# jynik/OOKiedokie

Measured on AMD Instinct MI355X. Metric: IQ Msamples/s demodulated (SC16Q11->bits), higher is better.
Workload: dtype f32

## Files before the change

### include/ookiedokie_amd.h

```cpp
#ifndef OOKIEDOKIE_AMD_H
#define OOKIEDOKIE_AMD_H

#include <limits.h>
#include <stddef.h>
#include <stdint.h>

#ifdef __cplusplus
extern "C" {
#endif

#define OOKD_API_VERSION 1

#define OOKD_FILE_EOF INT_MIN

enum {
    OOKD_OK = 0,
    OOKD_ERR_ARG = -1,
    OOKD_ERR_IO = -2,
    OOKD_ERR_PARSE = -3,
    OOKD_ERR_HIP = -4,
    OOKD_ERR_CAPACITY = -5,
    OOKD_ERR_NOMEM = -6
};

// ... 170 lines not shown
                           uint64_t capture_stride_samples);

int ookd_rx_submit_device(ookd_rx *rx, const void *d_iq,
                          uint32_t num_captures,
                          uint64_t samples_per_capture,
                          uint64_t capture_stride_samples);
int ookd_rx_wait(ookd_rx *rx);

int ookd_rx_process_host(ookd_rx *rx, const int16_t *iq,
                         uint64_t num_samples);

int ookd_rx_shard_begin(ookd_rx *rx, const void *d_iq, uint64_t num_samples,
                        const int16_t *halo, uint64_t halo_samples,
                        int last_shard, const ookd_fsm_state *state_in,
                        ookd_fsm_state *state_out);
int ookd_rx_shard_refine(ookd_rx *rx, const ookd_fsm_state *state_in,
                         ookd_fsm_state *state_out);
uint64_t ookd_rx_halo_samples(const ookd_rx *rx);

int ookd_scan_domain_info(const ookd_device *device,
                          uint32_t samples_per_buffer,
                          uint32_t total_decimation, uint32_t out[8]);

uint64_t ookd_rx_num_messages(const ookd_rx *rx);
const ookd_message *ookd_rx_messages(const ookd_rx *rx);
int ookd_rx_get_stats(const ookd_rx *rx, ookd_rx_stats *out);
int ookd_rx_get_front_info(const ookd_rx *rx, ookd_front_info *out);

uint64_t ookd_rx_bit_words(const ookd_rx *rx);
int ookd_rx_get_bits(const ookd_rx *rx, uint32_t capture, uint64_t *words,
                     uint64_t capacity_words);
int ookd_rx_get_edges(const ookd_rx *rx, uint32_t capture, uint64_t *edges,
                      uint64_t capacity, uint64_t *num_edges);
int ookd_rx_get_fir(const ookd_rx *rx, uint32_t capture, ookd_complexf *out,
                    uint64_t capacity);
int ookd_rx_get_errors(const ookd_rx *rx, uint64_t *samples, uint64_t capacity,
                       uint64_t *num);

size_t ookd_rx_dig_text(const ookd_rx *rx, uint32_t capture, char *out, size_t capacity);
int ookd_rx_record_dig(const ookd_rx *rx, uint32_t capture, const char *path);
int ookd_rx_get_fir_sc16q11(const ookd_rx *rx, uint32_t capture, int16_t *out,
                            uint64_t capacity_samples);
int ookd_rx_record_fir(const ookd_rx *rx, uint32_t capture, const char *path);

#define OOKD_LEVEL_BINS 256
typedef struct ookd_level_hist {
// ... 157 lines not shown
```

### ookiedokie_amd/__init__.py

```python
from __future__ import annotations

import ctypes as C
import os
from dataclasses import dataclass
from typing import List, Optional, Sequence, Tuple

import numpy as np

_HERE = os.path.dirname(os.path.abspath(__file__))
LIB_PATH = os.path.join(_HERE, "lib", "libookiedokie_amd.so")
HEADER_PATH = os.path.join(_HERE, "..", "include", "ookiedokie_amd.h")

MAX_PAYLOAD_BYTES = 32
FILE_EOF = -(2 ** 31)
RX_EXACT_FIR = 1
RX_KEEP_FIR = 2
RX_FSM_ROUNDS = 4
RX_NO_QUIET_SKIP = 8
RX_COUNT_QUIET = 16
RX_SCAN_SIMS = 32
RX_NO_PIPELINE = 128
RX_FIR_VALU = 256
RX_SCAN_TABLES = 512
RX_SAMPLES_CS8 = 1024
# ... 151 lines not shown
    "ookd_filter_load": (C.c_void_p, [C.c_char_p]),
    "ookd_filter_create": (C.c_void_p, [C.c_uint32, C.c_void_p, C.c_void_p, C.c_void_p]),
    "ookd_filter_free": (None, [C.c_void_p]),
    "ookd_filter_total_decimation": (C.c_uint32, [C.c_void_p]),
    "ookd_filter_num_stages": (C.c_uint32, [C.c_void_p]),
    "ookd_filter_stage": (C.c_int, [C.c_void_p, C.c_uint32, C.POINTER(C.c_uint32),
                                    C.POINTER(C.c_uint32), C.POINTER(C.POINTER(C.c_float))]),
    "ookd_filter_tuned_taps": (C.c_int, [C.c_void_p, C.c_double, C.c_uint32, C.c_void_p, C.c_void_p]),
    "ookd_device_load": (C.c_void_p, [C.c_char_p, C.c_uint32]),
    "ookd_device_create": (C.c_void_p, [C.POINTER(FsmTables)]),
    "ookd_device_free": (None, [C.c_void_p]),
    "ookd_device_num_bits": (C.c_uint32, [C.c_void_p]),
    "ookd_device_name": (C.c_char_p, [C.c_void_p]),
    "ookd_device_state_name": (C.c_char_p, [C.c_void_p, C.c_uint32]),
    "ookd_device_tables": (C.c_int, [C.c_void_p, C.POINTER(FsmTables)]),
    "ookd_rx_create": (C.c_void_p, [C.POINTER(RxConfig), C.c_void_p, C.c_void_p]),
    "ookd_rx_create_tuned": (C.c_void_p, [C.POINTER(RxConfig), C.c_void_p, C.c_void_p, C.POINTER(Tune)]),
    "ookd_rx_tune": (C.c_double, [C.c_void_p]),
    "ookd_rx_destroy": (None, [C.c_void_p]),
    "ookd_rx_sample_bytes": (C.c_uint32, [C.c_void_p]),
    "ookd_rx_process_device": (C.c_int, [C.c_void_p, C.c_void_p, C.c_uint32, C.c_uint64, C.c_uint64]),
    "ookd_rx_submit_device": (C.c_int, [C.c_void_p, C.c_void_p, C.c_uint32, C.c_uint64, C.c_uint64]),
    "ookd_scan_domain_info": (C.c_int, [C.c_void_p, C.c_uint32, C.c_uint32, C.POINTER(C.c_uint32)]),
    "ookd_rx_wait": (C.c_int, [C.c_void_p]),
    "ookd_rx_process_host": (C.c_int, [C.c_void_p, C.c_void_p, C.c_uint64]),
    "ookd_rx_shard_begin": (C.c_int, [C.c_void_p, C.c_void_p, C.c_uint64, C.c_void_p, C.c_uint64,
                                      C.c_int, C.POINTER(FsmState), C.POINTER(FsmState)]),
    "ookd_rx_shard_refine": (C.c_int, [C.c_void_p, C.POINTER(FsmState), C.POINTER(FsmState)]),
    "ookd_rx_halo_samples": (C.c_uint64, [C.c_void_p]),
    "ookd_rx_num_messages": (C.c_uint64, [C.c_void_p]),
    "ookd_rx_messages": (C.POINTER(Message), [C.c_void_p]),
    "ookd_rx_get_stats": (C.c_int, [C.c_void_p, C.POINTER(RxStats)]),
    "ookd_rx_get_front_info": (C.c_int, [C.c_void_p, C.POINTER(FrontInfo)]),
    "ookd_rx_bit_words": (C.c_uint64, [C.c_void_p]),
    "ookd_rx_get_bits": (C.c_int, [C.c_void_p, C.c_uint32, C.c_void_p, C.c_uint64]),
    "ookd_rx_get_edges": (C.c_int, [C.c_void_p, C.c_uint32, C.c_void_p, C.c_uint64,
                                    C.POINTER(C.c_uint64)]),
    "ookd_rx_get_fir": (C.c_int, [C.c_void_p, C.c_uint32, C.c_void_p, C.c_uint64]),
    "ookd_rx_get_errors": (C.c_int, [C.c_void_p, C.c_void_p, C.c_uint64, C.POINTER(C.c_uint64)]),
    "ookd_fir_create": (C.c_void_p, [C.c_int32, C.c_void_p, C.c_size_t, C.c_uint32]),
    "ookd_fir_reset": (None, [C.c_void_p]),
    "ookd_fir_destroy": (None, [C.c_void_p]),
    "ookd_fir_filter_and_decimate": (C.c_size_t, [C.c_void_p, C.c_void_p, C.c_size_t, C.c_void_p]),
    "ookd_synth_create": (C.c_void_p, [C.c_void_p, C.POINTER(SynthConfig), C.c_uint64]),
    "ookd_synth_free": (None, [C.c_void_p]),
    "ookd_synth_num_messages": (C.c_uint64, [C.c_void_p]),
# ... 843 lines not shown
```

### ookiedokie_amd/csrc/fir_mfma.hip

```cpp
#include "kernels.hpp"
#include "common.hpp"

#include <hip/hip_ext.h>

#include <algorithm>
#include <cmath>
#include <cstring>
#include <type_traits>

#pragma clang fp contract(off)

namespace ookd {

typedef _Float16 h8 __attribute__((ext_vector_type(8)));
typedef _Float16 h4 __attribute__((ext_vector_type(4)));
typedef float f16x __attribute__((ext_vector_type(16)));
typedef float v2fm __attribute__((ext_vector_type(2)));
typedef short v2s __attribute__((ext_vector_type(2)));
typedef uint32_t v4u __attribute__((ext_vector_type(4)));

__host__ __device__ constexpr uint32_t mslot(uint32_t j) { return j + 8u * (j >> 5); }

template <int KS, int FMT = (int)kFmtSc16>
struct MfmaGeom {
// ... 294 lines not shown
        are = __builtin_amdgcn_mfma_f32_32x32x16_f16(a1, xr, are, 0, 0, 0);
        aim = __builtin_amdgcn_mfma_f32_32x32x16_f16(a1, xi, aim, 0, 0, 0);
        __builtin_amdgcn_sched_barrier(0);
        xr = xr_n;
        xi = xi_n;
        a0 = a0_n;
        a1 = a1_n;
    }
    __builtin_amdgcn_fence(__ATOMIC_RELEASE, "wavefront");
    __builtin_amdgcn_wave_barrier();
}

template <int KS>
__device__ __noinline__ void mfma_fetch_image(const void *image, unsigned char *smem, uint32_t tid) {
    v4u *dst = reinterpret_cast<v4u *>(smem) + tid;
    const gptr128 src = reinterpret_cast<gptr128>((gbytes)image) + tid;
    for (int i = 0; i < 2 * KS; i += 4) {
        const v4u f0 = src[64 * i], f1 = src[64 * i + 64], f2 = src[64 * i + 128], f3 = src[64 * i + 192];
        dst[64 * i] = f0;
        dst[64 * i + 64] = f1;
        dst[64 * i + 128] = f2;
        dst[64 * i + 192] = f3;
    }
}

template <int KS, int FMT>
__global__ __launch_bounds__(64 * mfma_waves<KS>()) __attribute__((amdgpu_waves_per_eu(4)))
void fir1_mfma_kernel(const FrontParams p) {
    constexpr int kMfmaWaves = mfma_waves<KS>();
    extern __shared__ __attribute__((aligned(16))) unsigned char smem_raw[];
    using Gm = MfmaGeom<KS, FMT>;
    typedef typename RawSrcT<FMT>::elem raw_t;
    typedef typename RawSrcT<FMT>::ptr raw_ptr;
    constexpr uint32_t kImgBytes = (uint32_t)KS * 2u * 1024u;
    uint32_t tid = threadIdx.x & 63u;
    const uint32_t wave = threadIdx.x >> 6;
    const uint32_t cap = blockIdx.y;
    MfmaTileCtxT<FMT> c;
    c.rs.src = (raw_ptr)(reinterpret_cast<const raw_t *>(p.iq) + (uint64_t)cap * p.cap_stride);
    c.rs.halo = (raw_ptr)reinterpret_cast<const raw_t *>(p.halo);
    c.rs.halo_len = p.halo_len;
    c.rs.n_valid = p.n_valid;
    c.ctl = reinterpret_cast<uint32_t *>(smem_raw + kImgBytes);
    c.tickets = p.mfma_g * (uint32_t)kMfmaWaves;
    c.tile_base = p.tile_base;
    c.tile_end = p.tile_end;
// ... 61 lines not shown
                mfma_fetch_image<KS>(p.mfma_a, smem_raw, tid);
                __builtin_amdgcn_fence(__ATOMIC_RELEASE, "wavefront");
                __builtin_amdgcn_wave_barrier();
                if (tid == 0) __hip_atomic_store(&c.ctl[1], 1u, __ATOMIC_RELAXED, __HIP_MEMORY_SCOPE_WORKGROUP);
                __builtin_amdgcn_fence(__ATOMIC_ACQUIRE, "wavefront");
            }
            f16x are, aim;
            if (FMT != (int)kFmtSc16 || !wide) {
                mfma_convert<KS, FMT>(q, 0xffffffffu, tid, pl_re, pl_im);
                more = mfma_take_ticket(c, tid, tile_n);
                pre = more && mfma_interior<KS, FMT>(c, tile_n);
                if (pre) mfma_issue_loads<KS, FMT>(c, tile_n, tid, q);
                mfma_ksteps<KS, true>(a_img, pl_re, pl_im, tid, are, aim);
            } else if constexpr (FMT == (int)kFmtSc16) {
                mfma_convert<KS, FMT>(q, 0xffe0ffe0u, tid, pl_re, pl_im);
                mfma_ksteps<KS, true>(a_img, pl_re, pl_im, tid, are, aim);
                mfma_convert<KS, FMT>(q, 0x001f001fu, tid, pl_re, pl_im);
                more = mfma_take_ticket(c, tid, tile_n);
                pre = more && mfma_interior<KS, FMT>(c, tile_n);
                if (pre) mfma_issue_loads<KS, FMT>(c, tile_n, tid, q);
                mfma_ksteps<KS, false>(a_img, pl_re, pl_im, tid, are, aim);
            }

            const float plo = wide ? p.p_lo_w : p.p_lo_n;
            const float phi = wide ? p.p_hi_w : p.p_hi_n;
            const uint32_t ocol = 32u * n + 4u * hh;
            uint32_t m16 = 0;
            uint64_t any_unsure = 0;
#pragma unroll
            for (int r2 = 7; r2 >= 0; --r2) {
                const v2fm zr = (v2fm){are[2 * r2], are[2 * r2 + 1]}, zi = (v2fm){aim[2 * r2], aim[2 * r2 + 1]};
                const v2fm rr = zr * zr, ii = zi * zi;
                const v2fm pw = rr + ii;
                {
                    const uint64_t ge_hi = __ballot(pw.y >= phi);
                    asm("v_addc_co_u32_e64 %0, vcc, %0, %0, %1" : "+v"(m16) : "s"(ge_hi) : "vcc");
                    any_unsure |= __ballot(pw.y >= plo) & ~ge_hi;
                }
                {
                    const uint64_t ge_hi = __ballot(pw.x >= phi);
                    asm("v_addc_co_u32_e64 %0, vcc, %0, %0, %1" : "+v"(m16) : "s"(ge_hi) : "vcc");
                    any_unsure |= __ballot(pw.x >= plo) & ~ge_hi;
                }
            }
            if (any_unsure != 0) {
                uint32_t todo = 0, redo = 0;
#pragma unroll
                for (int r = 0; r < 16; ++r) {
                    const float rr = are[r] * are[r], ii = aim[r] * aim[r];
                    const float pw = rr + ii;
                    if (pw >= plo && !(pw >= phi)) todo |= 1u << r;
                }
                while (todo) {
                    const uint32_t r = (uint32_t)__ffs((int)todo) - 1u;
                    todo &= todo - 1u;
                    const uint64_t o = t0 + ocol + (r & 3u) + 8u * (r >> 2);
                    if (o >= p.n_out) continue;
                    const float2 y = mfma_exact_output(c.rs, (gptrf)p.taps, p.stage[0].ntaps, (int64_t)o);
                    const float rr = y.x * y.x, ii = y.y * y.y;
                    const float pe = rr + ii;
                    m16 = (m16 & ~(1u << r)) | ((pe >= p.p_star ? 1u : 0u) << r);
                    redo++;
                }
                if (redo && p.recompute_count) atomicAdd(p.recompute_count, (unsigned long long)redo);
            }
            if (fout) {
                const float cs = p.mfma_c;
#pragma unroll
                for (int r = 0; r < 16; ++r) {
                    const uint64_t o = t0 + ocol + (r & 3) + 8 * (r >> 2);
                    if (o < p.n_out) fout[o] = (v2fm){are[r] * cs, aim[r] * cs};
                }
            }

            uint32_t m32 = (m16 & 0xfu) | ((m16 & 0xf0u) << 4) | ((m16 & 0xf00u) << 8) | ((m16 & 0xf000u) << 12);
            m32 <<= 4u * hh;
            uint32_t w32 = m32 | (uint32_t)__shfl_xor((int)m32, 32);
            {
                const uint64_t c0 = t0 + 32u * n;
                if (c0 + 32u > p.n_out) {
                    const uint32_t keep = c0 >= p.n_out ? 0u : (uint32_t)(p.n_out - c0);
                    w32 &= (1u << keep) - 1u;
                }
            }
            {
                const uint32_t prev_top = (uint32_t)__shfl_up((int)(w32 >> 31), 1);
                uint32_t ch = w32 ^ (w32 << 1);
                if (n != 0) ch ^= prev_top & 1u;
                else ch &= ~1u;
                uint32_t cnt = hh == 0 ? (uint32_t)__popc(ch) : 0u;
#pragma unroll
                for (int d = 16; d >= 1; d >>= 1) cnt += (uint32_t)__shfl_xor((int)cnt, d);
                const uint32_t first = (uint32_t)__builtin_amdgcn_readfirstlane((int)(w32 & 1u));
                const uint32_t last = (uint32_t)__builtin_amdgcn_readlane((int)(w32 >> 31), 31);
                const uint64_t chl = __ballot(hh == 0 && ch != 0);
                const uint32_t widx = chl ? (uint32_t)__builtin_ctzll(chl) >> 1 : 0u;
                if (tid == 0) *uniform_ptr(tile_info + tile) = cnt | (widx << kTileWordShift) | (first << 30) | (last << 31) | p.stamp_bits;
            }
            const uint32_t up = (uint32_t)__shfl_xor((int)w32, 1);
            if (hh == 0 && (n & 1u) == 0) {
                const gbytes_w wb = uniform_ptr((gbytes_w)(words + (t0 >> 6)));
                *reinterpret_cast<gptr64>(wb + 4u * n) = (uint64_t)w32 | ((uint64_t)up << 32);
            }
        }

        if (!more) break;
        if (!pre) mfma_boundary_loads<KS, FMT>(c, tile_n, tid, win, q);
        tile = tile_n;
    }
}

constexpr uint32_t kF2Out = 256;
constexpr uint32_t kF2Tp = 96;
constexpr uint32_t kF2W = 4 * kF2Out + kF2Tp;
template <int FMT>
// ... 236 lines not shown
            if (__hip_atomic_load(&c.ctl[1], __ATOMIC_RELAXED, __HIP_MEMORY_SCOPE_WORKGROUP) == 0) {
                f2_fetch_image(p.mfma_a, smem_raw, tid);
                __builtin_amdgcn_fence(__ATOMIC_RELEASE, "wavefront");
                __builtin_amdgcn_wave_barrier();
                if (tid == 0) __hip_atomic_store(&c.ctl[1], 1u, __ATOMIC_RELAXED, __HIP_MEMORY_SCOPE_WORKGROUP);
                __builtin_amdgcn_fence(__ATOMIC_ACQUIRE, "wavefront");
            }
            f4x are, aim;
            if (FMT != (int)kFmtSc16 || !wide) {
                f2_convert<FMT>(q, 0xffffffffu, tid, pl_re, pl_im);
                more = mfma_take_ticket(c, tid, tile_n);
                pre = more && f2_interior(c, tile_n);
                if (pre) f2_issue_loads(c, tile_n, tid, q);
                f2_ksteps<true>(a_img, pl_re, pl_im, tid, are, aim);
            } else if constexpr (FMT == (int)kFmtSc16) {
                f2_convert<FMT>(q, 0xffe0ffe0u, tid, pl_re, pl_im);
                f2_ksteps<true>(a_img, pl_re, pl_im, tid, are, aim);
                f2_convert<FMT>(q, 0x001f001fu, tid, pl_re, pl_im);
                more = mfma_take_ticket(c, tid, tile_n);
                pre = more && f2_interior(c, tile_n);
                if (pre) f2_issue_loads(c, tile_n, tid, q);
                f2_ksteps<false>(a_img, pl_re, pl_im, tid, are, aim);
            }
            const float plo = wide ? p.p_lo_w : p.p_lo_n;
            const float phi = wide ? p.p_hi_w : p.p_hi_n;
            const uint32_t o_lane = 16u * n + 4u * g;
            uint32_t nib = 0, unsure = 0;
#pragma unroll
            for (int r = 0; r < 4; ++r) {
                const float rr = are[r] * are[r], ii = aim[r] * aim[r];
                const float pw = rr + ii;
                const bool hi = pw >= phi;
                nib |= (hi ? 1u : 0u) << r;
                unsure |= ((!hi && pw >= plo) ? 1u : 0u) << r;
            }
            if (__ballot(unsure != 0) != 0) {
                uint32_t todo = unsure, redo = 0;
                while (todo) {
                    const uint32_t r = (uint32_t)__ffs((int)todo) - 1u;
                    todo &= todo - 1u;
                    const uint64_t o = M0 + o_lane + r;
                    if (o >= p.n_out) continue;
                    const float2 y = fir2_mfma_exact_output(c.rs, ft, (int64_t)o);
                    const float rr = y.x * y.x, ii = y.y * y.y;
                    const float pe = rr + ii;
                    nib = (nib & ~(1u << r)) | ((pe >= p.p_star ? 1u : 0u) << r);
                    redo++;
                }
                if (redo && p.recompute_count) atomicAdd(p.recompute_count, (unsigned long long)redo);
            }
            if (fout) {
                const float cs = p.mfma_c;
#pragma unroll
                for (int r = 0; r < 4; ++r) {
                    const uint64_t o = M0 + o_lane + r;
                    if (o < p.n_out) fout[o] = (v2fm){are[r] * cs, aim[r] * cs};
                }
            }
            if (M0 + o_lane + 4u > p.n_out) {
                const uint32_t keep = M0 + o_lane >= p.n_out ? 0u : (uint32_t)(p.n_out - (M0 + o_lane));
                nib &= (1u << keep) - 1u;
            }
            uint64_t w64 = (uint64_t)nib << (16u * (n & 3u) + 4u * g);
#pragma unroll
            for (int d = 1; d <= 32; d <<= 1) {
                if (d == 4 || d == 8) continue;
                const uint32_t lo = (uint32_t)__shfl_xor((int)(uint32_t)w64, d), hi = (uint32_t)__shfl_xor((int)(uint32_t)(w64 >> 32), d);
                w64 |= (uint64_t)lo | ((uint64_t)hi << 32);
            }
            {
                const uint32_t wq = n >> 2;
                const uint32_t top_prev = (uint32_t)__shfl((int)(uint32_t)(w64 >> 63), (int)((wq ? wq - 1u : 0u) << 2));
                uint64_t ch = w64 ^ ((w64 << 1) | (wq ? (uint64_t)(top_prev & 1u) : 0ull));
                if (wq == 0) ch &= ~1ull;
                uint32_t cnt = ((n & 3u) == 0 && g == 0) ? (uint32_t)__popcll(ch) : 0u;
#pragma unroll
                for (int d = 32; d >= 1; d >>= 1) cnt += (uint32_t)__shfl_xor((int)cnt, d);
                const uint32_t first = (uint32_t)__builtin_amdgcn_readfirstlane((int)(uint32_t)(w64 & 1ull));
                const uint32_t last = (uint32_t)__builtin_amdgcn_readlane((int)(uint32_t)(w64 >> 63), 12);
                const uint64_t chl = __ballot((n & 3u) == 0 && g == 0 && ch != 0);
                const uint32_t widx = chl ? (uint32_t)__builtin_ctzll(chl) >> 2 : 0u;
                if (tid == 0) *uniform_ptr(tile_info + tile) = cnt | (widx << kTileWordShift) | (first << 30) | (last << 31) | p.stamp_bits;
            }
            if ((n & 3u) == 0 && g == 0) {
                const gbytes_w wb = uniform_ptr((gbytes_w)(words + (M0 >> 6)));
                *reinterpret_cast<gptr64>(wb + 2u * n) = w64;
            }
        }

        if (!more) break;
        if (!pre) f2_boundary_loads(c, tile_n, tid, win, q);
        tile = tile_n;
    }
}


static uint16_t half_bits(_Float16 h) {
    uint16_t b;
    std::memcpy(&b, &h, 2);
    return b;
// ... 125 lines not shown
    out.delta = delta;
    out.sum_abs = sum_abs;
    out.sum_hat = sum_hat;
    return true;
}

double mfma_error_bound2(const MfmaTaps &t, double e_ref, bool wide) {
    const double u = std::ldexp(1.0, -24);
    const double xmax = wide ? 16.0 : 1.0;
    const double chain = (double)t.ksteps * 32.0 * 2.0 * (wide ? 2.0 : 1.0);
    const double e_acc = chain * 2.0 * u * t.sum_hat;
    return 1.1 * (e_ref + (e_acc + t.delta) * xmax) + 78.0 * std::ldexp(1.0, -140);
}

double mfma_error_bound(const MfmaTaps &t, uint32_t ntaps, bool wide) {
    const double u = std::ldexp(1.0, -24);
    const double xmax = wide ? 16.0 : 1.0;
    const double chain = (double)t.ksteps * 16.0 * 2.0 * (wide ? 2.0 : 1.0);
    const double e_ref = ((double)ntaps + 1.0) * u * t.sum_abs;
    const double e_acc = chain * 2.0 * u * t.sum_hat;
    return 1.1 * (e_ref + e_acc + t.delta) * xmax + (double)ntaps * std::ldexp(1.0, -140);
}

bool mfma_scale_band(const MfmaTaps &t, float p, float &out) {
    if (std::isnan(p) || std::isinf(p) || p == 0.0f) {
        out = p;
        return true;
    }
    int e = 0;
    (void)std::frexp((double)t.c, &e);
    const double scaled = std::ldexp((double)p, -2 * (e - 1));
    const float f = (float)scaled;
    if (!std::isfinite(f) || (double)f != scaled || std::fabs(f) < 1.1754944e-38f) return false;
    out = f;
    return true;
}

bool front_uses_mfma(const FrontParams &p) {
    return p.mfma_a != nullptr && p.num_stages == 1 && p.stage[0].decim == 1 && p.origin == 0 && !p.iq_f32 &&
           mfma_ksteps_for(p.stage[0].ntaps) != 0;
}

bool front_uses_mfma2(const FrontParams &p) {
    return p.mfma_a != nullptr && p.num_stages == 2 && !p.iq_f32 && !p.halo_f32 && p.stage[0].decim == 2 &&
           p.stage[1].decim == 2 && p.stage[0].ntaps <= 16 && p.stage[1].ntaps <= 32 && p.origin % 4 == 0;
}

hipError_t launch_front_mfma2(const FrontParams &p, uint32_t num_captures, hipStream_t stream, hipEvent_t t0,
                              hipEvent_t t1, uint64_t tile_begin, uint64_t tile_count) {
    const uint64_t all = (p.n_out + kF2Out - 1) / kF2Out;
    const uint64_t b = tile_begin < all ? tile_begin : all;
    const uint64_t cnt = tile_count < all - b ? tile_count : all - b;
    if (cnt == 0) return hipSuccess;
    FrontParams pp = p;
    pp.tile_base = (uint32_t)b;
    pp.tile_end = b + cnt;
    if (pp.mfma_g == 0) pp.mfma_g = 1;
// ... 49 lines not shown
```

### ookiedokie_amd/csrc/kernels.hpp

```cpp
#pragma once

#include <hip/hip_runtime.h>

#include <vector>

#include <cstdint>

namespace ookd {

constexpr int kMaxStages = 8;
constexpr int kTapChunk = 32;
constexpr int kFirThreads = 256;
constexpr int kFirR = 16;
constexpr int kFirTile = kFirThreads * kFirR;
constexpr int kFirWaves = kFirThreads / 64;
constexpr int kFirWgWaves = 1;
constexpr int kFir1RShort = 8, kFir1RLong = 16;
constexpr uint32_t kFir1ShortTaps = 256;
constexpr int kWaveTile = 64 * kFirR;
constexpr int kQuietCounters = 1024;
constexpr int kGenTile = 1024;
constexpr int kBlockWords = 64;
constexpr int kPayloadWords = 5;

// ... 13 lines not shown
    uint64_t n_out;
    uint64_t origin;
    const int16_t *halo;
    const float *halo_f32;
    uint32_t halo_len;
    uint32_t num_stages;
    FirStageDev stage[kMaxStages];
    const float *taps;
    uint64_t *bits;
    uint64_t words_per_cap;
    float *fir_out;
    float p_star;
    float p_lo, p_hi;
    int quiet_lsb;
    unsigned long long *recompute_count;
    uint32_t *quiet_count;
    uint32_t *tile_info;
    uint32_t tiles_per_cap;
    uint32_t tile_base;
    uint32_t sparse;
    uint32_t stamp_bits;
    const void *mfma_a;
    float mfma_c;
    float p_lo_n, p_hi_n;
    float p_lo_w, p_hi_w;
    uint32_t mfma_g;
    uint32_t mfma_xcd;
    uint32_t mfma_xcd_span;
    uint64_t tile_end;
    uint32_t mfma_debug;
    uint32_t sample_fmt;
    uint32_t tune;
    const float *ctaps;
    float quiet_a, quiet_b;
};

enum : uint32_t { kFmtSc16 = 0, kFmtCs8 = 1, kFmtCu8 = 2 };
constexpr uint32_t sample_bytes(uint32_t fmt) { return fmt == kFmtSc16 ? 4u : 2u; }

#ifdef __HIPCC__
template <int FMT>
__device__ __forceinline__ uint32_t widen8(uint32_t s) {
    int i = (int)(s & 0xffu), q = (int)((s >> 8) & 0xffu);
    if (FMT == (int)kFmtCu8) {
        i -= 128;
        q -= 128;
    } else {
        i = (int)(int8_t)i;
// ... 9 lines not shown
constexpr uint32_t kTileStampShift = 14;
constexpr uint32_t kTileStampMask = 0x3fffc000u;
constexpr uint32_t kTileStampMax = 0xffffu;
__host__ __device__ __forceinline__ uint32_t tile_live(uint32_t info, uint32_t stamp_bits) {
    return ((info ^ stamp_bits) & kTileStampMask) ? 0u : (info & ~kTileStampMask);
}

hipError_t launch_clear_tiles(uint32_t *tile_info, uint64_t *bits, uint64_t ntiles, uint32_t tiles_per_cap,
                              uint64_t words_per_cap, uint32_t tile_bits, uint32_t keep_stamp_bits, hipStream_t stream);
bool front_sparse_capable(const FrontParams &p);

constexpr uint32_t kMfmaTile = 1024;

struct MfmaTaps {
    std::vector<uint16_t> image;
    uint32_t ksteps = 0;
    float c = 0.0f;
    double delta = 0.0;
    double sum_abs = 0.0;
    double sum_hat = 0.0;
};
bool mfma_prepare_taps(const float *taps, uint32_t ntaps, MfmaTaps &out);
double mfma_error_bound(const MfmaTaps &t, uint32_t ntaps, bool wide);
bool mfma_scale_band(const MfmaTaps &t, float p, float &out);
bool front_uses_mfma(const FrontParams &p);
bool mfma_prepare_taps2(const float *taps1, uint32_t n1, const float *taps2, uint32_t n2, MfmaTaps &out);
double mfma_error_bound2(const MfmaTaps &t, double e_ref, bool wide);
bool front_uses_mfma2(const FrontParams &p);
hipError_t launch_front_mfma2(const FrontParams &p, uint32_t num_captures, hipStream_t stream, hipEvent_t t0,
                              hipEvent_t t1, uint64_t tile_begin, uint64_t tile_count);
hipError_t launch_front_mfma(const FrontParams &p, uint32_t num_captures, hipStream_t stream, hipEvent_t t0,
                             hipEvent_t t1, uint64_t tile_begin, uint64_t tile_count);

hipError_t ensure_dynamic_lds(const void *func, size_t bytes);

hipError_t launch_front(const FrontParams &p, uint32_t num_captures, bool exact, hipStream_t stream,
                        hipEvent_t t0 = nullptr, hipEvent_t t1 = nullptr, uint64_t tile_begin = 0,
                        uint64_t tile_count = ~0ull);
uint32_t front_form(const FrontParams &p, bool exact);
uint64_t front_wave_tiles(const FrontParams &p);
uint32_t front_tile_bits(const FrontParams &p);
bool front_uses_tuned_fir1(const FrontParams &p);
uint32_t tuned_fir1_tile_bits(const FrontParams &p);
hipError_t launch_front_tuned_fir1(const FrontParams &p, uint32_t num_captures, hipStream_t stream, hipEvent_t t0,
                                   hipEvent_t t1, uint64_t tile_begin, uint64_t tile_count);
hipError_t launch_front_tuned_generic(const FrontParams &p, uint32_t num_captures, hipStream_t stream);
hipError_t launch_front_generic(const FrontParams &p, uint32_t num_captures,
// ... 324 lines not shown
```

### ookiedokie_amd/csrc/rx.cpp

```cpp
#include <algorithm>
#include <atomic>
#include <cerrno>
#include <chrono>
#include <cinttypes>
#include <cmath>
#include <cstddef>
#include <cstdlib>
#include <cstring>
#include <memory>
#include <mutex>
#include <utility>

#include "common.hpp"
#include "ingest.hpp"
#include "kernels.hpp"

using namespace ookd;

namespace {

#define HIPCHK(expr)                                                              \
    do {                                                                          \
        hipError_t _e = (expr);                                                   \
        if (_e != hipSuccess) {                                                   \
// ... 275 lines not shown
        if (ev_end) (void)hipEventDestroy(ev_end);
        if (s_front) (void)hipStreamDestroy(s_front);
        if (s_chain) (void)hipStreamDestroy(s_chain);
        if (h_hdr) (void)hipHostFree(h_hdr);
        if (h_msgs) (void)hipHostFree(h_msgs);
        for (hipEvent_t e : ev) if (e) (void)hipEventDestroy(e);
        if (own_stream && stream) (void)hipStreamDestroy(stream);
    }
};

}

struct ookd_rx : RxHandles {
    ookd_rx_config cfg{};

    uint32_t num_stages = 0;
    FirStageDev stage[kMaxStages]{};
    uint32_t total_decim = 1;
    uint64_t halo_needed = 0;
    std::vector<float> taps0;
    DevBuf<float> d_taps;
    float p_star = 0, p_lo = 0, p_hi = 0;
    DevBuf<uint16_t> d_mfma_a;
    float mfma_c = 0, p_lo_n = 0, p_hi_n = 0, p_lo_w = 0, p_hi_w = 0;
    uint32_t mfma_g = 0;
    uint32_t mfma_xcd = 2;
    double err_n = 0, err_w = 0, err_valu = 0, mfma_delta = 0;
    uint32_t mfma_ksteps = 0;
    uint32_t run_form = 0;
    int quiet_lsb = 0;
    double tune_nu = 0.0;
    DevBuf<float> d_ctaps;
    float quiet_a = 0, quiet_b = 0;
    uint32_t tile_bits = 0;
    bool exact = false;
    bool count_quiet = false;
    DevBuf<uint32_t> d_quiet;
    std::vector<uint32_t> quiet_prev;
    DevBuf<uint32_t> d_tile_info;
    bool sparse = false;
    uint64_t dirty_tiles = 0, dirty_words_per_cap = 0;
    uint32_t dirty_tiles_per_cap = 0;
    uint32_t tile_stamp = 0;
    mutable bool bits_dense = false;
    int densify_bits() const;
    bool pipe_ok = false;
    uint64_t pipe_chunk_in = 0;
// ... 110 lines not shown
        blocks = (uint32_t)(words / kBlockWords);
        segs = (uint32_t)((n_out + seg_len - 1) / seg_len);
        if (segs == 0 && n_out > 0) segs = 1;
    }

    FrontParams front_params(const void *d_iq, uint64_t stride) const {
        FrontParams p{};
        p.iq = static_cast<const int16_t *>(d_iq);
        p.cap_stride = stride;
        p.n_valid = run_n_valid;
        p.n_in = run_n_in;
        p.n_out = run_n_out;
        p.num_stages = num_stages;
        for (uint32_t s = 0; s < num_stages; ++s) p.stage[s] = stage[s];
        p.taps = d_taps.p;
        p.bits = d_bits.p;
        p.words_per_cap = run_words;
        p.fir_out = (cfg.flags & OOKD_RX_KEEP_FIR) ? d_fir.p : nullptr;
        p.p_star = p_star;
        p.p_lo = p_lo;
        p.p_hi = p_hi;
        p.mfma_a = d_mfma_a.p;
        p.mfma_c = mfma_c;
        p.p_lo_n = p_lo_n;
        p.p_hi_n = p_hi_n;
        p.p_lo_w = p_lo_w;
        p.p_hi_w = p_hi_w;
        p.mfma_g = mfma_g;
        p.mfma_xcd = mfma_xcd;
        {
            static const uint32_t dbg = dev_getenv("OOKD_MFMA_DEBUG") ? (uint32_t)atoi(dev_getenv("OOKD_MFMA_DEBUG")) : 0u;
            p.mfma_debug = dbg;
        }
        p.recompute_count = &d_hdr.p->recompute;
        p.quiet_lsb = quiet_lsb;
        p.quiet_count = count_quiet ? d_quiet.p : nullptr;
        p.tile_info = d_tile_info.p;
        p.tiles_per_cap = tile_bits ? (uint32_t)(run_words * 64 / tile_bits) : 0;
        p.sparse = sparse ? 1u : 0u;
        p.stamp_bits = tile_stamp << kTileStampShift;
        p.sample_fmt = sample_fmt;
        p.tune = tune_nu != 0.0 ? (exact ? 2u : 1u) : 0u;
        p.ctaps = d_ctaps.p;
        p.quiet_a = quiet_a;
        p.quiet_b = quiet_b;
        return p;
    }

    EdgeParams edge_params() const {
        EdgeParams e{};
// ... 786 lines not shown
        taps_dev.insert(taps_dev.end(), st.taps.begin(), st.taps.end());
        taps_dev.resize(d.tap_off + d.ntaps_pad, 0.0f);
        rx.stage[s] = d;
        rx.halo_needed += (uint64_t)(d.ntaps - 1) * mult;
        mult *= d.decim;
    }
    rx.taps0 = filter.stages[0].taps;
    if (rx.d_taps.alloc(taps_dev.size()) != OOKD_OK) return false;
    if (hipMemcpy(rx.d_taps.p, taps_dev.data(), taps_dev.size() * sizeof(float), hipMemcpyHostToDevice) != hipSuccess) {
        set_error("tap upload failed");
        return false;
    }
    return true;
}

bool setup_mfma(ookd_rx &rx, const MfmaTaps &mt, double e_n, double e_w) {
    rx.err_n = e_n;
    rx.err_w = e_w;
    rx.mfma_ksteps = mt.ksteps;
    rx.mfma_delta = mt.delta;
    float lo_n, hi_n, lo_w, hi_w;
    band_from_error(e_n, rx.p_star, lo_n, hi_n);
    band_from_error(e_w, rx.p_star, lo_w, hi_w);
    if (!(mfma_scale_band(mt, lo_n, rx.p_lo_n) && mfma_scale_band(mt, hi_n, rx.p_hi_n) &&
          mfma_scale_band(mt, lo_w, rx.p_lo_w) && mfma_scale_band(mt, hi_w, rx.p_hi_w))) {
        return true;
    }
    if (rx.p_star > 0.0f && !(rx.p_star >= 0x1p-100f && rx.p_star <= 0x1p100f)) return true;
    if (rx.d_mfma_a.alloc(mt.image.size()) != OOKD_OK) return false;
    if (hipMemcpy(rx.d_mfma_a.p, mt.image.data(), mt.image.size() * sizeof(uint16_t), hipMemcpyHostToDevice) !=
        hipSuccess) {
        set_error("tap image upload failed");
        return false;
    }
    rx.mfma_c = mt.c;
    rx.mfma_g = mt.ksteps <= 6 ? 4u : mt.ksteps <= 10 ? 16u : 32u;
    if (const char *g = dev_getenv("OOKD_MFMA_G")) rx.mfma_g = (uint32_t)std::min(4096, std::max(1, atoi(g)));
    rx.mfma_xcd = 2u | (mt.ksteps >= 10 ? 1u : 0u);
    if (const char *x = dev_getenv("OOKD_MFMA_XCD")) rx.mfma_xcd = (uint32_t)atoi(x);
    return true;
}

bool setup_front_form(ookd_rx &rx, const ookd_filter &filter, uint32_t flags) {
    std::vector<std::vector<float>> st;
    for (const auto &f : filter.stages) st.push_back(f.taps);
    guard_band(st, rx.p_star, rx.p_lo, rx.p_hi);
    rx.err_valu = guard_error(st, 16.0);
    if ((flags & OOKD_RX_FIR_VALU) || dev_getenv("OOKD_FIR_VALU")) return true;
// ... 530 lines not shown
}

int ookd_rx_process_host(ookd_rx *rx, const int16_t *iq, uint64_t num_samples) {
    clear_error();
    if (!rx || (!iq && num_samples)) {
        set_error("ookd_rx_process_host: null argument");
        return OOKD_ERR_ARG;
    }
    if (num_samples > rx->max_samples) {
        set_error("capture of %llu samples exceeds max_samples %llu", (unsigned long long)num_samples,
                  (unsigned long long)rx->max_samples);
        return OOKD_ERR_ARG;
    }
    HIPCHK(hipSetDevice(rx->dev));
    if (!rx->d_stage_in.p) {
        int rc = rx->d_stage_in.alloc(rx->max_samples * (sample_bytes(rx->sample_fmt) / 2) + 8);
        if (rc != OOKD_OK) return rc;
    }
    if (num_samples && rx->ingest.from_host(iq, rx->d_stage_in.p, num_samples * sample_bytes(rx->sample_fmt)) < 0) return OOKD_ERR_HIP;
    return ookd_rx_process_device(rx, rx->d_stage_in.p, 1, num_samples, num_samples);
}

uint64_t ookd_rx_halo_samples(const ookd_rx *rx) { return rx ? rx->halo_needed : 0; }

int ookd_scan_domain_info(const ookd_device *device, uint32_t samples_per_buffer, uint32_t total_decimation,
                          uint32_t out[8]) {
    clear_error();
    if (!device || !out || !samples_per_buffer || !total_decimation) {
        set_error("ookd_scan_domain_info: bad argument");
        return OOKD_ERR_ARG;
    }
    std::unique_ptr<FsmTablesDev> t(new FsmTablesDev());
    memset(t.get(), 0, sizeof(FsmTablesDev));
    fill_fsm_tables(*device, *t);
    std::vector<uint32_t> off, n0, pk;
    std::vector<uint16_t> reach, stuck_src;
    std::vector<uint8_t> stuck_rows;
    const bool ok = build_leaf_tables(*t, samples_per_buffer, total_decimation, off, n0, pk, reach, stuck_src,
                                      stuck_rows);
    size_t zeros = 0;
    for (uint32_t v : pk) zeros += v == 0;
    const uint32_t S = (uint32_t)device->state_duration_us.size();
    bool merged_ok = true;
    if (ok && !n0.empty()) {
        const std::vector<uint32_t> m = build_merged_rows(S, off, n0, pk);
        auto lookup = [&](uint32_t row, uint32_t L, uint32_t n) -> uint32_t {
// ... 437 lines not shown
```

Measured before the change: 1.555 million.

## Classify MFMA FIR power bands with integer bit compares and DPP reductions

Replaces the per-output float compares and ballots against the low and high power thresholds with an integer subtraction on the float bit patterns. A funnel-shift accumulates the hi mask directly into the final interleaved bit positions, and a single unsigned max tells whether any lane landed in the uncertain band. The shuffle-based popcount reductions and the fir2 word assembly are replaced by DPP row sums, readlane, and fewer shuffles. Thresholds are now precomputed on the host as bit patterns, with added range checks that can disable the MFMA path. The trade-off is a more intricate bit trick whose correctness relies on the power values being non-negative and finite.

```diff
diff --git a/include/ookiedokie_amd.h b/include/ookiedokie_amd.h
--- a/include/ookiedokie_amd.h
+++ b/include/ookiedokie_amd.h
@@ -216,6 +216,9 @@
                           uint32_t samples_per_buffer,
                           uint32_t total_decimation, uint32_t out[8]);
 
+int ookd_mfma_band_bits(float mfma_c, double sum_hat, int wide, float p_lo,
+                        float p_hi, uint32_t out[2]);
+
 uint64_t ookd_rx_num_messages(const ookd_rx *rx);
 const ookd_message *ookd_rx_messages(const ookd_rx *rx);
 int ookd_rx_get_stats(const ookd_rx *rx, ookd_rx_stats *out);
diff --git a/ookiedokie_amd/__init__.py b/ookiedokie_amd/__init__.py
--- a/ookiedokie_amd/__init__.py
+++ b/ookiedokie_amd/__init__.py
@@ -197,6 +197,7 @@
     "ookd_rx_process_device": (C.c_int, [C.c_void_p, C.c_void_p, C.c_uint32, C.c_uint64, C.c_uint64]),
     "ookd_rx_submit_device": (C.c_int, [C.c_void_p, C.c_void_p, C.c_uint32, C.c_uint64, C.c_uint64]),
     "ookd_scan_domain_info": (C.c_int, [C.c_void_p, C.c_uint32, C.c_uint32, C.POINTER(C.c_uint32)]),
+    "ookd_mfma_band_bits": (C.c_int, [C.c_float, C.c_double, C.c_int, C.c_float, C.c_float, C.POINTER(C.c_uint32)]),
     "ookd_rx_wait": (C.c_int, [C.c_void_p]),
     "ookd_rx_process_host": (C.c_int, [C.c_void_p, C.c_void_p, C.c_uint64]),
     "ookd_rx_shard_begin": (C.c_int, [C.c_void_p, C.c_void_p, C.c_uint64, C.c_void_p, C.c_uint64,
diff --git a/ookiedokie_amd/csrc/fir_mfma.hip b/ookiedokie_amd/csrc/fir_mfma.hip
--- a/ookiedokie_amd/csrc/fir_mfma.hip
+++ b/ookiedokie_amd/csrc/fir_mfma.hip
@@ -340,6 +340,65 @@
         dst[64 * i + 128] = f2;
         dst[64 * i + 192] = f3;
     }
+}
+
+__host__ __device__ constexpr uint32_t band_pos(uint32_t r) { return (r & 3u) + 8u * (r >> 2); }
+
+template <int N, typename V>
+__device__ __forceinline__ uint32_t band_mask(const V &are, const V &aim, uint32_t hi_bits, uint32_t &umax) {
+    uint32_t acc = ~0u;
+    umax = 0;
+#pragma unroll
+    for (int r2 = N / 2 - 1; r2 >= 0; --r2) {
+        const v2fm zr = (v2fm){are[2 * r2], are[2 * r2 + 1]}, zi = (v2fm){aim[2 * r2], aim[2 * r2 + 1]};
+        const v2fm rr = zr * zr, ii = zi * zi;
+        const v2fm pw = rr + ii;
+        const uint32_t u1 = __float_as_uint(pw.y) - hi_bits, u0 = __float_as_uint(pw.x) - hi_bits;
+        acc = __builtin_amdgcn_alignbit(acc, u1, 31);
+        acc = __builtin_amdgcn_alignbit(acc, u0, 31);
+        umax = max(max(umax, u1), u0);
+        if ((r2 & 1) == 0 && r2 != 0) acc = __builtin_amdgcn_alignbit(acc, ~0u, 28);
+    }
+    return ~acc;
+}
+
+template <int N, typename V, typename Exact>
+__device__ __forceinline__ uint32_t band_bits(const V &are, const V &aim, uint32_t lo_bits, uint32_t hi_bits, float p_star,
+                                              unsigned long long *recompute_count, Exact exact) {
+    uint32_t umax;
+    uint32_t m = band_mask<N>(are, aim, hi_bits, umax);
+    if (__ballot(umax > ~(hi_bits - lo_bits)) != 0) {
+        const float plo = __uint_as_float(lo_bits), phi = __uint_as_float(hi_bits);
+        uint32_t todo = 0, redo = 0;
+#pragma unroll
+        for (int r = 0; r < N; ++r) {
+            const float rr = are[r] * are[r], ii = aim[r] * aim[r];
+            const float pw = rr + ii;
+            if (pw >= plo && !(pw >= phi)) todo |= 1u << r;
+        }
+        while (todo) {
+            const uint32_t r = (uint32_t)__ffs((int)todo) - 1u;
+            todo &= todo - 1u;
+            float2 y;
+            if (!exact(r, y)) continue;
+            const float rr = y.x * y.x, ii = y.y * y.y;
+            const float pe = rr + ii;
+            const uint32_t b = band_pos(r);
+            m = (m & ~(1u << b)) | ((pe >= p_star ? 1u : 0u) << b);
+            redo++;
+        }
+        recompute_count = uniform_ptr(recompute_count);
+        if (redo && recompute_count) atomicAdd(recompute_count, (unsigned long long)redo);
+    }
+    return m;
+}
+
+__device__ __forceinline__ uint32_t row_sum16(uint32_t x) {
+    x += (uint32_t)__builtin_amdgcn_update_dpp(0, (int)x, 0xb1, 0xf, 0xf, false);
+    x += (uint32_t)__builtin_amdgcn_update_dpp(0, (int)x, 0x4e, 0xf, 0xf, false);
+    x += (uint32_t)__builtin_amdgcn_update_dpp(0, (int)x, 0x141, 0xf, 0xf, false);
+    x += (uint32_t)__builtin_amdgcn_update_dpp(0, (int)x, 0x140, 0xf, 0xf, false);
+    return x;
 }
 
 template <int KS, int FMT>
@@ -447,48 +506,14 @@
                 mfma_ksteps<KS, false>(a_img, pl_re, pl_im, tid, are, aim);
             }
 
-            const float plo = wide ? p.p_lo_w : p.p_lo_n;
-            const float phi = wide ? p.p_hi_w : p.p_hi_n;
             const uint32_t ocol = 32u * n + 4u * hh;
-            uint32_t m16 = 0;
-            uint64_t any_unsure = 0;
-#pragma unroll
-            for (int r2 = 7; r2 >= 0; --r2) {
-                const v2fm zr = (v2fm){are[2 * r2], are[2 * r2 + 1]}, zi = (v2fm){aim[2 * r2], aim[2 * r2 + 1]};
-                const v2fm rr = zr * zr, ii = zi * zi;
-                const v2fm pw = rr + ii;
-                {
-                    const uint64_t ge_hi = __ballot(pw.y >= phi);
-                    asm("v_addc_co_u32_e64 %0, vcc, %0, %0, %1" : "+v"(m16) : "s"(ge_hi) : "vcc");
-                    any_unsure |= __ballot(pw.y >= plo) & ~ge_hi;
-                }
-                {
-                    const uint64_t ge_hi = __ballot(pw.x >= phi);
-                    asm("v_addc_co_u32_e64 %0, vcc, %0, %0, %1" : "+v"(m16) : "s"(ge_hi) : "vcc");
-                    any_unsure |= __ballot(pw.x >= plo) & ~ge_hi;
-                }
-            }
-            if (any_unsure != 0) {
-                uint32_t todo = 0, redo = 0;
-#pragma unroll
-                for (int r = 0; r < 16; ++r) {
-                    const float rr = are[r] * are[r], ii = aim[r] * aim[r];
-                    const float pw = rr + ii;
-                    if (pw >= plo && !(pw >= phi)) todo |= 1u << r;
-                }
-                while (todo) {
-                    const uint32_t r = (uint32_t)__ffs((int)todo) - 1u;
-                    todo &= todo - 1u;
-                    const uint64_t o = t0 + ocol + (r & 3u) + 8u * (r >> 2);
-                    if (o >= p.n_out) continue;
-                    const float2 y = mfma_exact_output(c.rs, (gptrf)p.taps, p.stage[0].ntaps, (int64_t)o);
-                    const float rr = y.x * y.x, ii = y.y * y.y;
-                    const float pe = rr + ii;
-                    m16 = (m16 & ~(1u << r)) | ((pe >= p.p_star ? 1u : 0u) << r);
-                    redo++;
-                }
-                if (redo && p.recompute_count) atomicAdd(p.recompute_count, (unsigned long long)redo);
-            }
+            uint32_t m32 = band_bits<16>(are, aim, wide ? p.lo_bits_w : p.lo_bits_n, wide ? p.hi_bits_w : p.hi_bits_n, p.p_star,
+                                         p.recompute_count, [&](uint32_t r, float2 &y) {
+                                             const uint64_t o = t0 + ocol + band_pos(r);
+                                             if (o >= p.n_out) return false;
+                                             y = mfma_exact_output(c.rs, (gptrf)p.taps, p.stage[0].ntaps, (int64_t)o);
+                                             return true;
+                                         });
             if (fout) {
                 const float cs = p.mfma_c;
 #pragma unroll
@@ -498,7 +523,6 @@
                 }
             }
 
-            uint32_t m32 = (m16 & 0xfu) | ((m16 & 0xf0u) << 4) | ((m16 & 0xf00u) << 8) | ((m16 & 0xf000u) << 12);
             m32 <<= 4u * hh;
             uint32_t w32 = m32 | (uint32_t)__shfl_xor((int)m32, 32);
             {
@@ -513,9 +537,8 @@
                 uint32_t ch = w32 ^ (w32 << 1);
                 if (n != 0) ch ^= prev_top & 1u;
                 else ch &= ~1u;
-                uint32_t cnt = hh == 0 ? (uint32_t)__popc(ch) : 0u;
-#pragma unroll
-                for (int d = 16; d >= 1; d >>= 1) cnt += (uint32_t)__shfl_xor((int)cnt, d);
+                const uint32_t rows = row_sum16(hh == 0 ? (uint32_t)__popc(ch) : 0u);
+                const uint32_t cnt = (uint32_t)__builtin_amdgcn_readlane((int)rows, 0) + (uint32_t)__builtin_amdgcn_readlane((int)rows, 16);
                 const uint32_t first = (uint32_t)__builtin_amdgcn_readfirstlane((int)(w32 & 1u));
                 const uint32_t last = (uint32_t)__builtin_amdgcn_readlane((int)(w32 >> 31), 31);
                 const uint64_t chl = __ballot(hh == 0 && ch != 0);
@@ -798,33 +821,14 @@
                 if (pre) f2_issue_loads(c, tile_n, tid, q);
                 f2_ksteps<false>(a_img, pl_re, pl_im, tid, are, aim);
             }
-            const float plo = wide ? p.p_lo_w : p.p_lo_n;
-            const float phi = wide ? p.p_hi_w : p.p_hi_n;
             const uint32_t o_lane = 16u * n + 4u * g;
-            uint32_t nib = 0, unsure = 0;
-#pragma unroll
-            for (int r = 0; r < 4; ++r) {
-                const float rr = are[r] * are[r], ii = aim[r] * aim[r];
-                const float pw = rr + ii;
-                const bool hi = pw >= phi;
-                nib |= (hi ? 1u : 0u) << r;
-                unsure |= ((!hi && pw >= plo) ? 1u : 0u) << r;
-            }
-            if (__ballot(unsure != 0) != 0) {
-                uint32_t todo = unsure, redo = 0;
-                while (todo) {
-                    const uint32_t r = (uint32_t)__ffs((int)todo) - 1u;
-                    todo &= todo - 1u;
-                    const uint64_t o = M0 + o_lane + r;
-                    if (o >= p.n_out) continue;
-                    const float2 y = fir2_mfma_exact_output(c.rs, ft, (int64_t)o);
-                    const float rr = y.x * y.x, ii = y.y * y.y;
-                    const float pe = rr + ii;
-                    nib = (nib & ~(1u << r)) | ((pe >= p.p_star ? 1u : 0u) << r);
-                    redo++;
-                }
-                if (redo && p.recompute_count) atomicAdd(p.recompute_count, (unsigned long long)redo);
-            }
+            uint32_t nib = band_bits<4>(are, aim, wide ? p.lo_bits_w : p.lo_bits_n, wide ? p.hi_bits_w : p.hi_bits_n, p.p_star,
+                                        p.recompute_count, [&](uint32_t r, float2 &y) {
+                                            const uint64_t o = M0 + o_lane + r;
+                                            if (o >= p.n_out) return false;
+                                            y = fir2_mfma_exact_output(c.rs, ft, (int64_t)o);
+                                            return true;
+                                        });
             if (fout) {
                 const float cs = p.mfma_c;
 #pragma unroll
@@ -837,21 +841,20 @@
                 const uint32_t keep = M0 + o_lane >= p.n_out ? 0u : (uint32_t)(p.n_out - (M0 + o_lane));
                 nib &= (1u << keep) - 1u;
             }
-            uint64_t w64 = (uint64_t)nib << (16u * (n & 3u) + 4u * g);
-#pragma unroll
-            for (int d = 1; d <= 32; d <<= 1) {
-                if (d == 4 || d == 8) continue;
-                const uint32_t lo = (uint32_t)__shfl_xor((int)(uint32_t)w64, d), hi = (uint32_t)__shfl_xor((int)(uint32_t)(w64 >> 32), d);
-                w64 |= (uint64_t)lo | ((uint64_t)hi << 32);
-            }
+            uint32_t h32 = nib << (4u * g);
+            h32 |= (uint32_t)__shfl_xor((int)h32, 16);
+            h32 |= (uint32_t)__shfl_xor((int)h32, 32);
+            h32 <<= 16u * (n & 1u);
+            h32 |= (uint32_t)__shfl_xor((int)h32, 1);
+            const uint32_t o32 = (uint32_t)__shfl_xor((int)h32, 2);
+            const uint64_t w64 = (n & 2u) ? (uint64_t)o32 | ((uint64_t)h32 << 32) : (uint64_t)h32 | ((uint64_t)o32 << 32);
             {
                 const uint32_t wq = n >> 2;
                 const uint32_t top_prev = (uint32_t)__shfl((int)(uint32_t)(w64 >> 63), (int)((wq ? wq - 1u : 0u) << 2));
                 uint64_t ch = w64 ^ ((w64 << 1) | (wq ? (uint64_t)(top_prev & 1u) : 0ull));
                 if (wq == 0) ch &= ~1ull;
-                uint32_t cnt = ((n & 3u) == 0 && g == 0) ? (uint32_t)__popcll(ch) : 0u;
-#pragma unroll
-                for (int d = 32; d >= 1; d >>= 1) cnt += (uint32_t)__shfl_xor((int)cnt, d);
+                const uint32_t cnt = (uint32_t)__builtin_amdgcn_readfirstlane(
+                    (int)row_sum16(((n & 3u) == 0 && g == 0) ? (uint32_t)__popcll(ch) : 0u));
                 const uint32_t first = (uint32_t)__builtin_amdgcn_readfirstlane((int)(uint32_t)(w64 & 1ull));
                 const uint32_t last = (uint32_t)__builtin_amdgcn_readlane((int)(uint32_t)(w64 >> 63), 12);
                 const uint64_t chl = __ballot((n & 3u) == 0 && g == 0 && ch != 0);
@@ -1023,7 +1026,7 @@
     return 1.1 * (e_ref + e_acc + t.delta) * xmax + (double)ntaps * std::ldexp(1.0, -140);
 }
 
-bool mfma_scale_band(const MfmaTaps &t, float p, float &out) {
+static bool mfma_scale_edge(const MfmaTaps &t, float p, float &out) {
     if (std::isnan(p) || std::isinf(p) || p == 0.0f) {
         out = p;
         return true;
@@ -1034,6 +1037,27 @@
     const float f = (float)scaled;
     if (!std::isfinite(f) || (double)f != scaled || std::fabs(f) < 1.1754944e-38f) return false;
     out = f;
+    return true;
+}
+
+bool mfma_scale_band(const MfmaTaps &t, float p_lo, float p_hi, bool wide, uint32_t &lo_bits, uint32_t &hi_bits) {
+    lo_bits = hi_bits = 0;
+    float lo = 0.0f, hi = 0.0f;
+    if (!mfma_scale_edge(t, p_lo, lo) || !mfma_scale_edge(t, p_hi, hi)) return false;
+    if (!(t.c > 0.0f) || !std::isfinite(t.c) || !std::isfinite(t.sum_hat)) return false;
+    const double zmax = t.sum_hat * (wide ? 16.0 : 1.0) / (double)t.c;
+    if (!(2.0 * zmax * zmax * (1.0 + 0x1p-10) < 0x1p127)) return false;
+    const uint32_t kInf = 0x7f800000u;
+    auto bits = [](float f) {
+        uint32_t b;
+        std::memcpy(&b, &f, 4);
+        return b;
+    };
+    const uint32_t H = std::isnan(hi) ? kInf : hi <= 0.0f ? 0u : bits(hi);
+    const uint32_t L = std::isnan(lo) ? H : lo <= 0.0f ? 0u : bits(lo);
+    if (L > H) return false;
+    lo_bits = L;
+    hi_bits = H;
     return true;
 }
 
diff --git a/ookiedokie_amd/csrc/kernels.hpp b/ookiedokie_amd/csrc/kernels.hpp
--- a/ookiedokie_amd/csrc/kernels.hpp
+++ b/ookiedokie_amd/csrc/kernels.hpp
@@ -59,8 +59,8 @@
     uint32_t stamp_bits;
     const void *mfma_a;
     float mfma_c;
-    float p_lo_n, p_hi_n;
-    float p_lo_w, p_hi_w;
+    uint32_t lo_bits_n, hi_bits_n;
+    uint32_t lo_bits_w, hi_bits_w;
     uint32_t mfma_g;
     uint32_t mfma_xcd;
     uint32_t mfma_xcd_span;
@@ -116,7 +116,7 @@
 };
 bool mfma_prepare_taps(const float *taps, uint32_t ntaps, MfmaTaps &out);
 double mfma_error_bound(const MfmaTaps &t, uint32_t ntaps, bool wide);
-bool mfma_scale_band(const MfmaTaps &t, float p, float &out);
+bool mfma_scale_band(const MfmaTaps &t, float p_lo, float p_hi, bool wide, uint32_t &lo_bits, uint32_t &hi_bits);
 bool front_uses_mfma(const FrontParams &p);
 bool mfma_prepare_taps2(const float *taps1, uint32_t n1, const float *taps2, uint32_t n2, MfmaTaps &out);
 double mfma_error_bound2(const MfmaTaps &t, double e_ref, bool wide);
diff --git a/ookiedokie_amd/csrc/rx.cpp b/ookiedokie_amd/csrc/rx.cpp
--- a/ookiedokie_amd/csrc/rx.cpp
+++ b/ookiedokie_amd/csrc/rx.cpp
@@ -321,7 +321,8 @@
     DevBuf<float> d_taps;
     float p_star = 0, p_lo = 0, p_hi = 0;
     DevBuf<uint16_t> d_mfma_a;
-    float mfma_c = 0, p_lo_n = 0, p_hi_n = 0, p_lo_w = 0, p_hi_w = 0;
+    float mfma_c = 0;
+    uint32_t lo_bits_n = 0, hi_bits_n = 0, lo_bits_w = 0, hi_bits_w = 0;
     uint32_t mfma_g = 0;
     uint32_t mfma_xcd = 2;
     double err_n = 0, err_w = 0, err_valu = 0, mfma_delta = 0;
@@ -478,10 +479,10 @@
         p.p_hi = p_hi;
         p.mfma_a = d_mfma_a.p;
         p.mfma_c = mfma_c;
-        p.p_lo_n = p_lo_n;
-        p.p_hi_n = p_hi_n;
-        p.p_lo_w = p_lo_w;
-        p.p_hi_w = p_hi_w;
+        p.lo_bits_n = lo_bits_n;
+        p.hi_bits_n = hi_bits_n;
+        p.lo_bits_w = lo_bits_w;
+        p.hi_bits_w = hi_bits_w;
         p.mfma_g = mfma_g;
         p.mfma_xcd = mfma_xcd;
         {
@@ -1314,8 +1315,8 @@
     float lo_n, hi_n, lo_w, hi_w;
     band_from_error(e_n, rx.p_star, lo_n, hi_n);
     band_from_error(e_w, rx.p_star, lo_w, hi_w);
-    if (!(mfma_scale_band(mt, lo_n, rx.p_lo_n) && mfma_scale_band(mt, hi_n, rx.p_hi_n) &&
-          mfma_scale_band(mt, lo_w, rx.p_lo_w) && mfma_scale_band(mt, hi_w, rx.p_hi_w))) {
+    if (!(mfma_scale_band(mt, lo_n, hi_n, false, rx.lo_bits_n, rx.hi_bits_n) &&
+          mfma_scale_band(mt, lo_w, hi_w, true, rx.lo_bits_w, rx.hi_bits_w))) {
         return true;
     }
     if (rx.p_star > 0.0f && !(rx.p_star >= 0x1p-100f && rx.p_star <= 0x1p100f)) return true;
@@ -1892,6 +1893,18 @@
 }
 
 uint64_t ookd_rx_halo_samples(const ookd_rx *rx) { return rx ? rx->halo_needed : 0; }
+
+int ookd_mfma_band_bits(float mfma_c, double sum_hat, int wide, float p_lo, float p_hi, uint32_t out[2]) {
+    clear_error();
+    if (!out) {
+        set_error("ookd_mfma_band_bits: bad argument");
+        return OOKD_ERR_ARG;
+    }
+    MfmaTaps t;
+    t.c = mfma_c;
+    t.sum_hat = sum_hat;
+    return mfma_scale_band(t, p_lo, p_hi, wide != 0, out[0], out[1]) ? 1 : 0;
+}
 
 int ookd_scan_domain_info(const ookd_device *device, uint32_t samples_per_buffer, uint32_t total_decimation,
                           uint32_t out[8]) {
```

Result: no change. 1.586 million, median of 4 (+2.0%).
